# edp1096/toy-spice

Measured on NVIDIA B200. Metric: circuit-timesteps/sec (batched FP64 transient), higher is better.
Workload: dtype f64

## Files before the change

### toy-spice_b200/csrc/device/skeleton.cuh

```cuda
#ifndef TSB_SKELETON_CUH
#define TSB_SKELETON_CUH

#define TSB_MAX_VARYING 128
#define TSB_UC_MAX 32

struct TsbArgs {
    long long n_inst;
    const double* pv[TSB_MAX_VARYING];
    const double* U;
    int analysis;
    int uic;
    double tstart, tstop, tstep, maxstep, minstep;
    int max_iter;
    double abstol, reltol, trtol;
    int out_flags;
    long long cap_rows;
    double* wave;
    double* stats;
    long long* rows;
    int* status;
    long long* counters;
    double* scratch;
    const double* sweep;
    int n_sweep;
// ... 92 lines not shown
    long long inst;
    long long n_rows;
    bool overflow;
    double2* sm;
    int grid_k;
    __device__ __forceinline__ TsbSink(const TsbArgs& a_, long long inst_) : a(a_), inst(inst_), n_rows(0), overflow(false), grid_k(0) {
        sm = reinterpret_cast<double2*>(tsb_smem) + threadIdx.x;
    }
    __device__ __forceinline__ void begin(long long inst_) {
        inst = inst_; n_rows = 0; overflow = false; grid_k = 0;
        if (a.out_flags & TSB_OUT_STATS) {
#pragma unroll
            for (int j = 0; j < NCOL; ++j) {
                sm[(2 * j) * TSB_BLOCK] = make_double2(__longlong_as_double(0x7ff0000000000000LL),
                                                       __longlong_as_double(0xfff0000000000000LL));
                sm[(2 * j + 1) * TSB_BLOCK] = make_double2(0.0, 0.0);
            }
        }
    }
    __device__ __forceinline__ double grid_time(int k) const {
        const double t = __dadd_rn(a.tstart, __dmul_rn((double)(k + 1), a.grid_dt));
        return t < a.tstop ? t : a.tstop;
    }
    __device__ __forceinline__ void emit_grid(const double* row) {
        const double t1 = row[0];
        while (grid_k < a.n_grid) {
            const double tg = grid_time(grid_k);
            if (tg > t1) break;
            double w = 1.0;
            if (n_rows > 0) { const double t0 = sm[1 * TSB_BLOCK].y; w = (tg - t0) / (t1 - t0); }
            double* o = a.wave + ((long long)grid_k * NCOL) * a.n_inst + inst;
            __stcs(o, tg);
#pragma unroll
            for (int j = 1; j < NCOL; ++j) {
                const double v0 = n_rows > 0 ? sm[(2 * j + 1) * TSB_BLOCK].y : row[j];
                __stcs(o + j * a.n_inst, v0 + (row[j] - v0) * w);
            }
            ++grid_k;
        }
    }
    __device__ __forceinline__ void push(const double* row) {
        if (TSB_GRID && (a.out_flags & TSB_OUT_GRID)) emit_grid(row);
        if (a.out_flags & TSB_OUT_WAVE) {
            if (n_rows < a.cap_rows) {
                double* w = a.wave + (n_rows * NCOL) * a.n_inst + inst;
#pragma unroll
                for (int j = 0; j < NCOL; ++j) __stcs(w + j * a.n_inst, row[j]);
            } else overflow = true;
        }
        if (a.out_flags & TSB_OUT_STATS) {
            if (n_rows == 0) sm[0] = make_double2(row[0], row[0]);
            bool grow = !TSB_X_GROW;
#pragma unroll
            for (int j = 1; TSB_X_GROW && j < NCOL; ++j) {
                const double2 mm = sm[(2 * j) * TSB_BLOCK];
                grow |= (row[j] < mm.x) | (row[j] > mm.y);
            }
            if (grow) {
#pragma unroll
                for (int j = 1; j < NCOL; ++j) {
                    const double v = row[j];
                    double2 mm = sm[(2 * j) * TSB_BLOCK];
                    if (TSB_X_STATS_PRED) {
                        double* slot = reinterpret_cast<double*>(&sm[(2 * j) * TSB_BLOCK]);
                        if (v < mm.x) slot[0] = v;
                        if (v > mm.y) slot[1] = v;
                    } else {
                        mm.x = v < mm.x ? v : mm.x;
                        mm.y = v > mm.y ? v : mm.y;
                        sm[(2 * j) * TSB_BLOCK] = mm;
                    }
                }
            }
#pragma unroll
            for (int j = 0; j < NCOL; ++j) {
                double2 sl = sm[(2 * j + 1) * TSB_BLOCK];
                sl.x += row[j];
                sl.y = row[j];
                sm[(2 * j + 1) * TSB_BLOCK] = sl;
            }
        }
        ++n_rows;
    }
    __device__ __forceinline__ void finish(bool ok = true) {
        if (TSB_GRID && (a.out_flags & TSB_OUT_GRID) && ok && n_rows > 0) {
            while (grid_k < a.n_grid) {
                double* o = a.wave + ((long long)grid_k * NCOL) * a.n_inst + inst;
                __stcs(o, grid_time(grid_k));
#pragma unroll
                for (int j = 1; j < NCOL; ++j) __stcs(o + j * a.n_inst, sm[(2 * j + 1) * TSB_BLOCK].y);
                ++grid_k;
            }
        }
        if (a.out_flags & TSB_OUT_STATS) {
#pragma unroll
            for (int j = 0; j < NCOL; ++j) {
                double2 mm = sm[(2 * j) * TSB_BLOCK];
                const double2 sl = sm[(2 * j + 1) * TSB_BLOCK];
                if (j == 0 && n_rows > 0) {
                    const double f = mm.x, l = sl.y;
                    mm.x = f < l ? f : l; mm.y = f < l ? l : f;
                }
                a.stats[(long long)(0 * NCOL + j) * a.n_inst + inst] = mm.x;
                a.stats[(long long)(1 * NCOL + j) * a.n_inst + inst] = mm.y;
                a.stats[(long long)(2 * NCOL + j) * a.n_inst + inst] = sl.x;
                a.stats[(long long)(3 * NCOL + j) * a.n_inst + inst] = sl.y;
            }
        }
        a.rows[inst] = (TSB_GRID && (a.out_flags & TSB_OUT_GRID)) ? (long long)grid_k : n_rows;
    }
};

#ifndef TSB_TGRID
#define TSB_TGRID 0
#endif
#ifndef TSB_X_TG_EARLY
#define TSB_X_TG_EARLY 1
#endif
#define TSB_TG_HDR 3
#define TSB_TG_NO_KEY (-3.0)
template <int NSRC> struct TsbTgLayout { static constexpr int ND = ((TSB_TG_HDR + NSRC + 1) / 2) * 2; };
__device__ __forceinline__ unsigned long long tsb_ld_acquire(const unsigned long long* p) {
    unsigned long long v;
    asm volatile("ld.acquire.gpu.global.u64 %0, [%1];" : "=l"(v) : "l"(p) : "memory");
    return v;
}
__device__ __forceinline__ void tsb_st_release(unsigned long long* p, unsigned long long v) {
    asm volatile("st.release.gpu.global.u64 [%0], %1;" ::"l"(p), "l"(v) : "memory");
}
__device__ __forceinline__ unsigned long long tsb_ld_relaxed(const unsigned long long* p) {
    unsigned long long v;
    asm volatile("ld.relaxed.gpu.global.u64 %0, [%1];" : "=l"(v) : "l"(p) : "memory");
    return v;
}
__device__ __forceinline__ void tsb_fence_acquire() { asm volatile("fence.acq_rel.gpu;" ::: "memory"); }
__device__ __forceinline__ void tsb_prefetch_l1(const void* p) { asm volatile("prefetch.global.L1 [%0];" ::"l"(p)); }
#ifndef TSB_TG_PUBLISH_EVERY
#define TSB_TG_PUBLISH_EVERY 8
#endif
#ifndef TSB_TG_LOOK_EVERY
#define TSB_TG_LOOK_EVERY 16
#endif
#ifndef TSB_TG_CACHED
#define TSB_TG_CACHED 0
#endif
#ifndef TSB_TG_PREFETCH
#define TSB_TG_PREFETCH 0
#endif
#if TSB_TG_CACHED
#define TSB_TG_LD(p) __ldca(p)
#else
#define TSB_TG_LD(p) __ldcg(p)
#endif

template <bool HAVE_KEY = false, bool HAVE_SMALL = false, class Ckt, class Sink>
__device__ __forceinline__ void tsb_accept_step(const TsbArgs& a, Ckt& c, Sink& sink, double& time, double& dt,
                                                double next_time, double lte, TsbTimeKeyer& keyer, double& last_key, double key_in = 0.0,
                                                bool lte_small = false) {
    c.load_state(dt);
    c.update_state();
    time = next_time;
    if (time >= a.tstart) {
        double key = HAVE_KEY ? key_in : keyer.key(time);
        if (key != last_key) {
            double row[Ckt::NCOL_MAX];
            row[0] = time;
            c.signals(row + 1);
            sink.push(row);
            last_key = key;
        }
    }
    if (time < a.tstop && dt < a.maxstep) {
        const double grown = (HAVE_SMALL ? lte_small : lte < a.trtol / 100) ? dt * 2 : dt * 1.1;
        dt = grown < a.maxstep ? grown : a.maxstep;
    }
}

template <class Ckt, class Sink>
__device__ __forceinline__ void tsb_tran_linear(const TsbArgs& a, Ckt& c, Sink& sink, long long& n_acc_out, long long& n_rej_out,
                                                long long& n_sol_tran_out, long long& n_exec_out, int& status, double& fail_at) {
    double time = 0.0, dt = a.minstep;
    double last_key = -1.0;
    TsbTimeKeyer keyer; keyer.reset();
    int n_acc = 0, n_rej = 0, n_bad = 0;
    constexpr int ND = TsbTgLayout<Ckt::NSRC>::ND;
    const bool tg_pub = TSB_TGRID && a.tgrid != nullptr && a.tgrid_role == 1;
    const bool tg_reader = TSB_TGRID && a.tgrid != nullptr && a.tgrid_role == 0;
    int tg_limit = TSB_X_TGLOOK ? 0 : (tg_reader ? 0 : -1);
    int tg_next = tg_reader ? 0 : 0x7fffffff;
#if TSB_X_UNROLL2
#pragma unroll 2
#endif
    while (time < a.tstop) {
        const int k = n_acc + n_rej;
        const double t_tag = time, dt_tag = dt;
        bool look = false;
        if (TSB_TGRID && TSB_X_TGLOOK) {
            if (k == tg_next) {
                const unsigned long long pub = tsb_ld_relaxed(a.tgrid_pub);
                const int lim = pub < (unsigned long long)a.tgrid_cap ? (int)pub : a.tgrid_cap;
                if (lim > k) { tsb_fence_acquire(); tg_limit = lim; tg_next = (lim + TSB_TG_LOOK_EVERY - 1) & ~(TSB_TG_LOOK_EVERY - 1); }
                else tg_next = k + TSB_TG_LOOK_EVERY;
                if (k >= a.tgrid_cap) { tg_limit = 0; tg_next = 0x7fffffff; }
            }
            look = k < tg_limit;
        } else if (TSB_TGRID && tg_limit >= 0) {
            if (k >= tg_limit && (k & (TSB_TG_LOOK_EVERY - 1)) == 0) {
                const unsigned long long pub = tsb_ld_relaxed(a.tgrid_pub);
                const int lim = pub < (unsigned long long)a.tgrid_cap ? (int)pub : a.tgrid_cap;
                if (lim > k) { tsb_fence_acquire(); tg_limit = lim; }
                if (k >= a.tgrid_cap) tg_limit = -1;
            }
            look = k < tg_limit;
            if (TSB_TG_PREFETCH && look) tsb_prefetch_l1(a.tgrid + (long long)k * ND);
        }
#if TSB_X_TGLOOK
        double2 e0, e1;
#else
        double2 e0 = make_double2(0.0, 0.0), e1 = make_double2(0.0, 0.0);
#endif
        if (TSB_TGRID && TSB_X_TG_EARLY && look) {
            const double2* e = reinterpret_cast<const double2*>(a.tgrid + (long long)k * ND);
            e0 = TSB_TG_LD(e); e1 = TSB_TG_LD(e + 1);
        }
        double next_time = time + dt;
        if (next_time > a.tstop) { next_time = a.tstop; dt = next_time - time; }
        __builtin_assume(dt > 0.0);
        const double rdt = tsb_rcp_dt(dt);
        double lte = 0.0;
        bool lte_gt, lte_small;
        if (TSB_X_LTEFLAGS) c.lte_flags(dt, rdt, a.trtol, a.trtol / 100, lte_gt, lte_small);
        else { lte = c.lte(dt, rdt); lte_gt = lte > a.trtol; lte_small = lte < a.trtol / 100; }
        if (lte_gt && dt > a.minstep) {
            if (tg_pub && k < a.tgrid_cap) {
                double2* e = reinterpret_cast<double2*>(a.tgrid + (long long)k * ND);
                __stcg(e, make_double2(t_tag, dt_tag));
                __stcg(e + 1, make_double2(TSB_TG_NO_KEY, 0.0));
                if ((k & (TSB_TG_PUBLISH_EVERY - 1)) == TSB_TG_PUBLISH_EVERY - 1) tsb_st_release(a.tgrid_pub, (unsigned long long)k + 1);
            }
            dt /= 2; ++n_rej; continue;
        }
        double key = 0.0;
        auto mid = [&]() {
            bool hit = false;
            if (TSB_TGRID && look) {
                const double2* e = reinterpret_cast<const double2*>(a.tgrid + (long long)k * ND);
                if (!TSB_X_TG_EARLY) { e0 = TSB_TG_LD(e); e1 = TSB_TG_LD(e + 1); }
                hit = ((__double_as_longlong(e0.x) ^ __double_as_longlong(t_tag)) | (__double_as_longlong(e0.y) ^ __double_as_longlong(dt_tag))) == 0;
                if (!hit) { tg_limit = TSB_X_TGLOOK ? 0 : -1; tg_next = 0x7fffffff; }
                hit = hit && e1.x != TSB_TG_NO_KEY;
                if (hit) {
                    key = e1.x;
                    if (Ckt::SRC_UNIFORM) {
                        c.SV[0] = e1.y;
#pragma unroll
                        for (int j = 1; j < Ckt::NSRC; j += 2) {
                            const double2 sv = TSB_TG_LD(e + 2 + j / 2);
                            c.SV[j] = sv.x;
                            if (j + 1 < Ckt::NSRC) c.SV[j + 1] = sv.y;
                        }
                    }
                }
            }
            if (!hit || !Ckt::SRC_UNIFORM) { if (!c.eval_sources_nb(time)) c.eval_sources(time, 1.0); }
            if (!hit) key = next_time >= a.tstart ? keyer.key_any(next_time) : -2.0;
            if (tg_pub && k < a.tgrid_cap) {
                double2* e = reinterpret_cast<double2*>(a.tgrid + (long long)k * ND);
                __stcg(e, make_double2(t_tag, dt_tag));
                __stcg(e + 1, make_double2(key, c.SV[0]));
#pragma unroll
                for (int j = 1; j < Ckt::NSRC; j += 2) __stcg(e + 2 + j / 2, make_double2(c.SV[j], j + 1 < Ckt::NSRC ? c.SV[j + 1] : 0.0));
                if ((k & (TSB_TG_PUBLISH_EVERY - 1)) == TSB_TG_PUBLISH_EVERY - 1) tsb_st_release(a.tgrid_pub, (unsigned long long)k + 1);
            }
        };
        bool solved;
        if constexpr (Ckt::HAS_TF) solved = c.template assemble_solve_tf<false>(time, dt, rdt, mid);
        else solved = c.template assemble_solve<TSB_MODE_TRAN, false>(TSB_MODE_TRAN, time, dt, rdt, 0.0, mid);
        if (!solved) {
            ++n_bad;
            if (dt > a.minstep) { dt /= 2; ++n_rej; continue; }
            status = TSB_ST_TRAN_FAILED; fail_at = time;
            break;
        }
        tsb_accept_step<true, true>(a, c, sink, time, dt, next_time, lte, keyer, last_key, key, lte_small);
        ++n_acc;
    }
    if (tg_pub) { const int k = n_acc + n_rej; tsb_st_release(a.tgrid_pub, (unsigned long long)(k < a.tgrid_cap ? k : a.tgrid_cap)); }
    n_acc_out += n_acc; n_rej_out += n_rej;
    const int failed = status == TSB_ST_TRAN_FAILED ? 1 : 0;
    n_exec_out += n_acc + (n_bad - failed) + failed;
    n_sol_tran_out += 2LL * (n_acc + n_rej) - n_bad + 2 * failed;
}

#ifndef TSB_X_NLLOOP
#define TSB_X_NLLOOP 1
#endif
template <class Ckt, class Sink>
__device__ __forceinline__ void tsb_tran_nonlinear(const TsbArgs& a, Ckt& c, Sink& sink, bool active, long long& n_acc_out,
                                                   long long& n_rej_out, long long& n_sol_tran_out, long long& n_exec_out,
                                                   int& status, double& fail_at) {
    constexpr int N = Ckt::N;
    double time = 0.0, dt = a.minstep;
    double last_key = -1.0;
    TsbTimeKeyer keyer; keyer.reset();
    int n_acc = 0, n_rej = 0, n_sol = 0;
    bool live = active && time < a.tstop;
    while (__any_sync(0xffffffffu, live)) {
        double next_time = time + dt;
        if (next_time > a.tstop) { next_time = a.tstop; dt = next_time - time; }
        double rdt = 0.0;
        if (live) {
            if (!c.eval_sources_nb(time)) c.eval_sources(time, 1.0);
            rdt = tsb_rcp_dt(dt);
        }
        int iter = 0;
#if TSB_X_NRSTATE
        int nr = live ? 0 : 2;
        while (__any_sync(0xffffffffu, nr == 0)) {
            if (nr == 0) {
                if (iter > 0) c.update_nl(c.xo);
                bool solved;
                if constexpr (Ckt::HAS_TF) solved = c.template assemble_solve_tf<true>(time, dt, rdt, typename Ckt::TsbNoMid());
                else solved = c.template assemble_solve<TSB_MODE_TRAN>(TSB_MODE_TRAN, time, dt, rdt, 0.0);
                ++n_sol;
                if (!solved) nr = 2;
                else {
                    const bool cv = iter > 0 && tsb_converged<N>(c.x, c.xo, a.reltol, a.abstol);
                    if (cv) nr = 1;
                    else {
#pragma unroll
                        for (int i = 1; i <= N; ++i) c.xo[i] = c.x[i];
                        if (++iter >= a.max_iter) nr = 2;
                    }
                }
            }
        }
        const bool fail = nr == 2;
#else
        bool conv = false, fail = false, iterating = live;
        while (__any_sync(0xffffffffu, iterating)) {
            if (iterating) {
                if (iter > 0) c.update_nl(c.xo);
                bool solved;
                if constexpr (Ckt::HAS_TF) solved = c.template assemble_solve_tf<true>(time, dt, rdt, typename Ckt::TsbNoMid());
                else solved = c.template assemble_solve<TSB_MODE_TRAN>(TSB_MODE_TRAN, time, dt, rdt, 0.0);
                ++n_sol;
                if (!solved) fail = true;
                else {
                    if (iter > 0) conv = tsb_converged<N>(c.x, c.xo, a.reltol, a.abstol);
                    if (!conv) {
#pragma unroll
                        for (int i = 1; i <= N; ++i) c.xo[i] = c.x[i];
                        if (++iter >= a.max_iter) fail = true;
                    }
                }
                iterating = !(conv || fail);
            }
        }
#endif
        if (live) {
            if (fail) {
                if (dt > a.minstep) { dt /= 2; ++n_rej; }
                else { status = TSB_ST_TRAN_FAILED; fail_at = time; live = false; }
            } else {
                const double lte = c.lte(dt, rdt);
                if (lte > a.trtol && dt > a.minstep) { dt /= 2; ++n_rej; }
                else {
                    tsb_accept_step(a, c, sink, time, dt, next_time, lte, keyer, last_key);
                    ++n_acc;
                    live = time < a.tstop;
                }
            }
        }
    }
    n_acc_out += n_acc; n_rej_out += n_rej; n_sol_tran_out += n_sol; n_exec_out += n_sol;
}

#ifndef TSB_X_WSYNC
#define TSB_X_WSYNC 1
#endif
template <class Ckt>
__device__ __forceinline__ void tsb_run_optran_instance(const TsbArgs& a, long long inst, bool valid) {
    constexpr int N = Ckt::N;
    constexpr bool LINEAR_LOOP = !Ckt::HAS_NL && (TSB_SKIP_LINEAR_RESOLVE != 0);
    constexpr bool REFILL = Ckt::HAS_NL && (TSB_LANE_REFILL != 0);
    constexpr bool WSYNC = Ckt::HAS_NL && !REFILL && (TSB_X_WSYNC != 0);
    constexpr bool NL_LOOP = WSYNC && (TSB_X_NLLOOP != 0);
    if (!WSYNC && !valid) return;
    Ckt c;
    TsbSink<Ckt::NCOL_MAX> sink(a, inst);

    long long n_acc, n_rej, n_sol_tran, n_sol_op;
    long long n_exec;
    int op_path, status;
    double fail_at;

    enum { PH_OP_START, PH_TRAN_BEGIN, PH_NR, PH_DONE };
    enum { C_MAIN, C_GMIN, C_GFINAL, C_SRC, C_SFINAL, C_TRAN };
    int phase, op_pass, cont, iter, mode, gstep;
    double gmin, sfac, status_dt;
    double time, dt, next_time, rdt;
    double last_key;
    TsbTimeKeyer keyer;
    bool linear_tran;

    auto begin_instance = [&]() {
        c.load(a, inst);
        c.init();
        if constexpr (Ckt::HAS_TF) c.prefactor();
        sink.begin(inst);
        n_acc = n_rej = n_sol_tran = n_sol_op = n_exec = 0;
        op_path = 0; status = TSB_ST_OK; fail_at = 0.0;
        phase = (a.analysis == TSB_AN_TRAN && a.uic) ? PH_TRAN_BEGIN : PH_OP_START;
        op_pass = 0; cont = C_MAIN; iter = 0; mode = TSB_MODE_OP; gstep = 0;
        gmin = 0.0; sfac = 0.0; status_dt = 0.0;
        time = 0.0; dt = a.minstep; next_time = 0.0; rdt = 0.0;
        last_key = -1.0; keyer.reset();
        linear_tran = false;
        if (phase == PH_TRAN_BEGIN && !(time < a.tstop)) phase = PH_DONE;
        if ((LINEAR_LOOP || NL_LOOP) && phase == PH_TRAN_BEGIN) { linear_tran = true; phase = PH_DONE; }
    };
    auto finish_instance = [&]() {
        if (sink.overflow && status == TSB_ST_OK) status = TSB_ST_OVERFLOW;
        if (a.analysis == TSB_AN_OP) a.rows[inst] = sink.n_rows; else sink.finish(status == TSB_ST_OK);
        a.status[inst] = status;
        a.counters[0 * a.n_inst + inst] = n_acc;
        a.counters[1 * a.n_inst + inst] = n_rej;
        a.counters[2 * a.n_inst + inst] = n_sol_tran;
        a.counters[3 * a.n_inst + inst] = n_sol_op;
        a.counters[4 * a.n_inst + inst] = op_path;
        a.counters[5 * a.n_inst + inst] = __double_as_longlong(fail_at);
        a.counters[6 * a.n_inst + inst] = n_exec;
        a.counters[7 * a.n_inst + inst] = sink.n_rows;
    };
    bool done = !valid;
    bool pend = false;
    bool conv = false, fail = false;
    phase = PH_DONE;
    if (valid) begin_instance();
// ... 270 lines not shown
```

### toy-spice_b200/csrc/runtime.cpp

```cpp
#include <cuda_runtime.h>
#include <dlfcn.h>
#include <sys/stat.h>
#include <unistd.h>
#include <atomic>
#include <cmath>
#include <cstdio>
#include <cstdlib>
#include <cstring>
#include <fstream>
#include <memory>
#include <mutex>
#include <sstream>
#include "tsb_internal.hpp"
#include "hostlu.hpp"

namespace tsb {
cudaError_t launch_fp64_peak(double* scratch, int blocks, int iters, cudaStream_t s);
cudaError_t launch_totals(const long long* counters, long long n_inst, unsigned long long* totals, int sms, cudaStream_t s);
cudaError_t launch_fill_i64(long long* p, long long n, long long v, int sms, cudaStream_t s);
cudaError_t launch_summary(const double* stats, long long n_inst, int ncol, double* partial, int blocks_x, cudaStream_t s);
cudaError_t launch_lu_warp(const double* A, const double* b, double* x, int* status, long long n_inst, int n, const int* prow,
                           const int* pcol, int strict, int sms, cudaStream_t s);
cudaError_t launch_clu_warp(const double* A, const double* b, double* x, int* status, long long n_inst, int n, const int* prow,
                            const int* pcol, int strict, int sms, cudaStream_t s);
// ... 919 lines not shown
    if ((d.kind == TSB_V || d.kind == TSB_I) && d.src_type() == TSB_SRC_PWL)
        return fail(b->ctx, TSB_E_UNSUPPORTED, "PWL tables are not sweepable");
    *flat = d.p_off + param;
    return TSB_OK;
}
static int claim_slot(tsb_batch* b, int flat) {
    if (b->var_slot[flat] >= 0) return b->var_slot[flat];
    b->varying[flat] = 1;
    b->var_slot[flat] = (int)b->slot_ptr.size();
    b->slot_ptr.push_back(nullptr);
    b->slot_owned.push_back(0);
    b->slot_stage.push_back(nullptr);
    b->slot_staged.push_back(nullptr);
    return b->var_slot[flat];
}
static int set_param_host(tsb_batch* b, int dev, int param, const double* values, bool staged) {
    int flat = 0, rc = param_index(b, dev, param, &flat);
    if (rc != TSB_OK) return rc;
    if (!values) return TSB_E_INVALID;
    int slot = claim_slot(b, flat);
    if (!b->ctx) return TSB_OK;
    tsb_ctx* ctx = b->ctx;
    CU(ctx, cudaSetDevice(ctx->device));
    const size_t bytes = (size_t)b->n_inst * sizeof(double);
    if (!b->slot_owned[slot]) {
        double* p = nullptr;
        CU(ctx, cudaMalloc(&p, bytes));
        b->slot_ptr[slot] = p; b->slot_owned[slot] = 1;
    }
    const double* src = values;
    if (staged) {
        if (!b->slot_stage[slot]) {
            CU(ctx, cudaMallocHost((void**)&b->slot_stage[slot], bytes));
            CU(ctx, cudaEventCreateWithFlags(&b->slot_staged[slot], cudaEventDisableTiming));
        } else CU(ctx, cudaEventSynchronize(b->slot_staged[slot]));
        memcpy(b->slot_stage[slot], values, bytes);
        src = b->slot_stage[slot];
    }
    cudaStream_t up = ctx->stream;
    cudaStreamCaptureStatus cap = cudaStreamCaptureStatusNone;
    if (cudaStreamIsCapturing(ctx->stream, &cap) != cudaSuccess) { cudaGetLastError(); cap = cudaStreamCaptureStatusNone; }
    const bool beside = cap == cudaStreamCaptureStatusNone;
    if (beside) {
        if (!ctx->upload_stream) CU(ctx, cudaStreamCreateWithFlags(&ctx->upload_stream, cudaStreamNonBlocking));
        up = ctx->upload_stream;
        if (b->ev_launched) CU(ctx, cudaStreamWaitEvent(up, b->ev_launched, 0));
    }
    CU(ctx, cudaMemcpyAsync(b->slot_ptr[slot], src, bytes, cudaMemcpyHostToDevice, up));
    if (staged) CU(ctx, cudaEventRecord(b->slot_staged[slot], up));
    if (beside) {
        if (!b->ev_params) CU(ctx, cudaEventCreateWithFlags(&b->ev_params, cudaEventDisableTiming));
        CU(ctx, cudaEventRecord(b->ev_params, up));
        b->params_pending = true;
    }
    return TSB_OK;
}
int tsb_batch_set_param(tsb_batch* b, int dev, int param, const double* values) { return set_param_host(b, dev, param, values, true); }
int tsb_batch_set_param_async(tsb_batch* b, int dev, int param, const double* values) { return set_param_host(b, dev, param, values, false); }
int tsb_batch_set_param_dev(tsb_batch* b, int dev, int param, uint64_t dev_ptr) {
    int flat = 0, rc = param_index(b, dev, param, &flat);
    if (rc != TSB_OK) return rc;
    if (!dev_ptr) return TSB_E_INVALID;
    int slot = claim_slot(b, flat);
    if (b->slot_owned[slot]) { cudaFree(b->slot_ptr[slot]); b->slot_owned[slot] = 0; }
    b->slot_ptr[slot] = (double*)(uintptr_t)dev_ptr;
    return TSB_OK;
}
int tsb_batch_set_param_uniform(tsb_batch* b, int dev, int param, double value) {
    int flat = 0, rc = param_index(b, dev, param, &flat);
    if (rc != TSB_OK) return rc;
    if (b->varying[flat]) return fail(b->ctx, TSB_E_INVALID, "parameter already set per instance");
    b->uniform[flat] = value;
    return TSB_OK;
}

int tsb_run_op(tsb_batch* b, const tsb_opts* opts) {
    int rc = check_batch(b); if (rc != TSB_OK) return rc;
    tsb_ctx* ctx = b->ctx;
    tsb_opts o = resolve(opts, b->plan->p);
    o.coop_parts = 0;
    CU(ctx, cudaSetDevice(ctx->device));
    KernelModule* m = nullptr;
    if ((rc = get_module(b, o, -1, &m)) != TSB_OK) return rc;
    if ((rc = alloc_results(b, TSB_AN_OP, TSB_OUT_WAVE, 1, 0)) != TSB_OK) return rc;
    TsbArgsHost a;
    if ((rc = fill_common(b, o, a)) != TSB_OK) return rc;
    a.analysis = TSB_AN_OP;
    return launch(b, o, m->optran, a, b->plan->p.has_nonlinear && o.lane_refill != 0, m->min_blocks);
}

int tsb_run_tran(tsb_batch* b, double tstart, double tstop, double tstep, double tmax, int uic, int out_flags,
                 int64_t wave_cap_rows, const tsb_opts* opts) {
    int rc = check_batch(b); if (rc != TSB_OK) return rc;
    tsb_ctx* ctx = b->ctx;
    if (!(tstop > 0) || !(tstep > 0)) return fail(ctx, TSB_E_INVALID, "tstop and tstep must be positive");
    if (!(out_flags & (TSB_OUT_WAVE | TSB_OUT_STATS | TSB_OUT_GRID))) return fail(ctx, TSB_E_INVALID, "no output selected");
    if ((out_flags & TSB_OUT_WAVE) && (out_flags & TSB_OUT_GRID)) return fail(ctx, TSB_E_INVALID, "TSB_OUT_WAVE and TSB_OUT_GRID share the waveform buffer: select one");
    if ((out_flags & TSB_OUT_WAVE) && wave_cap_rows <= 0) return fail(ctx, TSB_E_INVALID, "wave_cap_rows must be positive");
    tsb_opts o = resolve(opts, b->plan->p);
    if (tstep > tstop / 300) tstep = tstop / 300;
    double minstep = tstep / 50.0;
    if (tmax == 0) tmax = tstep;
    double grid_dt = 0.0; int64_t n_grid = 0;
    if (out_flags & TSB_OUT_GRID) {
        out_flags |= TSB_OUT_STATS;
        grid_dt = o.grid_dt > 0 ? o.grid_dt : tstep;
        double span = tstop - tstart;
        if (!(span > 0) || !(grid_dt > 0)) return fail(ctx, TSB_E_INVALID, "TSB_OUT_GRID needs tstart < tstop and a positive grid spacing");
        double q = span / grid_dt;
        if (q > 1e7) return fail(ctx, TSB_E_INVALID, "TSB_OUT_GRID: more than 1e7 grid points");
        n_grid = (int64_t)floor(q * (1.0 + 1e-12) + 1e-9);
        if (n_grid < 1) n_grid = 1;
        wave_cap_rows = n_grid;
    }
    CU(ctx, cudaSetDevice(ctx->device));
    if (const char* ce = getenv("TSB_COOP")) { if (*ce) o.coop_parts = atoi(ce); }
    if (o.coop_parts < 0) {
        const Plan& cpl = b->plan->p;
        o.coop_parts = 0;
        if (!cpl.has_bjt && !cpl.has_mutual && !o.strict_fp && !(out_flags & TSB_OUT_GRID) && o.skip_linear_resolve && !o.lane_refill) {
            if (cpl.n() >= TSB_COOP_AUTO_MIN_N)
                for (int pick : {2, 4, 8}) {
                    if (!cpl.coop.count(pick)) continue;
                    const int nx = cpl.coop.at(pick).nx, nown = cpl.coop.at(pick).nown_max;
                    if (((size_t)4 * nown * 32 * pick + (size_t)2 * pick * nx * 32) * sizeof(double) <= 110 * 1024) { o.coop_parts = pick; break; }
                }
        }
    }
    if (o.coop_parts != 0) {
        const Plan& cpl = b->plan->p;
        if (o.coop_parts != 2 && o.coop_parts != 4 && o.coop_parts != 8) return fail(ctx, TSB_E_INVALID, "coop_parts must be -1, 0, 2, 4 or 8");
        if (cpl.has_bjt || cpl.has_mutual) return fail(ctx, TSB_E_UNSUPPORTED, "coop_parts: circuits with BJTs or mutual couplings run thread-per-circuit");
        if (!cpl.coop.count(o.coop_parts)) return fail(ctx, TSB_E_UNSUPPORTED, "coop_parts: the netlist has no partition into that many sub-circuits (tsb_plan_coop_info)");
        if (o.strict_fp) return fail(ctx, TSB_E_UNSUPPORTED, "coop_parts: the nested-dissection order is a re-association, not available in the strict build");
        if (out_flags & TSB_OUT_GRID) return fail(ctx, TSB_E_UNSUPPORTED, "coop_parts: TSB_OUT_GRID is not available on the cooperative mapping");
        if (!o.skip_linear_resolve || o.lane_refill) return fail(ctx, TSB_E_UNSUPPORTED, "coop_parts needs skip_linear_resolve = 1 and lane_refill = 0");
        if (o.min_blocks <= 0) o.min_blocks = 2;
    } else fit_block_to_shared_memory(o, b->plan->p.num_columns(TSB_AN_TRAN), out_flags);
    KernelModule* m = nullptr;
    b->grid_kernel = (out_flags & TSB_OUT_GRID) != 0;
    std::string autokey;
    rc = get_module(b, o, -1, &m, &autokey);
    if (rc != TSB_OK) { b->grid_kernel = false; return rc; }
    if ((rc = alloc_results(b, TSB_AN_TRAN, out_flags, (out_flags & (TSB_OUT_WAVE | TSB_OUT_GRID)) ? wave_cap_rows : 0, 0)) != TSB_OK) return rc;
    TsbArgsHost a;
    if ((rc = fill_common(b, o, a)) != TSB_OK) return rc;
    a.analysis = TSB_AN_TRAN; a.uic = uic;
    a.tstart = tstart; a.tstop = tstop; a.tstep = tstep; a.maxstep = tmax; a.minstep = minstep;
    a.grid_dt = grid_dt; a.n_grid = (int)n_grid;
    const bool persistent = b->plan->p.has_nonlinear && o.lane_refill != 0;
    const char* tune_env = getenv("TSB_AUTOTUNE");
    cudaStreamCaptureStatus cap = cudaStreamCaptureStatusNone;
    if (cudaStreamIsCapturing(ctx->stream, &cap) != cudaSuccess) { cudaGetLastError(); cap = cudaStreamCaptureStatusNone; }
    if (o.coop_parts == 0 && o.min_blocks <= 0 && !autokey.empty() && b->n_inst >= TSB_TUNE_MIN_INSTANCES && !ctx->tuned.count(autokey) &&
        !(tune_env && *tune_env == '0') && cap == cudaStreamCaptureStatusNone) {
        rc = autotune_min_blocks(b, o, autokey, m->min_blocks, a, persistent);
        if (rc == TSB_OK) rc = get_module(b, o, -1, &m);
        if (rc != TSB_OK) { b->grid_kernel = false; return rc; }
    }
    b->grid_kernel = false;
    b->tgrid_used = 0;
    const Plan& pl = b->plan->p;
    if (o.coop_parts > 0) {
        if (!m->coop) return fail(ctx, TSB_E_COMPILE, "cooperative kernel missing from the module");
        const CoopPlan& cp = pl.coop.at(o.coop_parts);
        if (!b->d_coop_state) CU(ctx, cudaMalloc(&b->d_coop_state, (size_t)(pl.n_state + pl.n() + 1) * b->n_inst * sizeof(double)));
        a.coop_state = b->d_coop_state;
        TsbArgsHost a1 = a;
        a1.out_flags = 0;
        if ((rc = launch(b, o, m->optran, a1, false, m->min_blocks)) != TSB_OK) return rc;
        const int nx = cp.nx, nown = cp.nown_max;
        const int groups = 1, block = 32 * cp.parts * groups;
        const size_t smem = ((size_t)4 * nown * block + (size_t)groups * 2 * cp.parts * nx * 32) * sizeof(double);
        if (smem > 227 * 1024) return fail(ctx, TSB_E_UNSUPPORTED, "coop_parts: the statistics of one block do not fit in shared memory");
        if (smem > 48 * 1024) CU(ctx, cudaFuncSetAttribute((const void*)m->coop, cudaFuncAttributeMaxDynamicSharedMemorySize, (int)smem));
        long long blocks = (a.n_run + 32 * groups - 1) / (32 * groups);
        if (blocks > 0x7fffffffLL) blocks = 0x7fffffffLL;
        if (blocks < 1) blocks = 1;
        void* kargs[] = {&a};
        CU(ctx, cudaLaunchKernel((const void*)m->coop, dim3((unsigned)blocks), dim3((unsigned)block), kargs, smem, ctx->stream));
        ++ctx->launches;
        return note_launched(b);
    }
    const bool tg_possible = !pl.has_nonlinear && o.skip_linear_resolve != 0 && o.share_time_grid != 0 && !persistent;
    if (tg_possible && (o.share_time_grid > 0 || b->n_inst >= TSB_TGRID_MIN_INSTANCES)) {
        if ((rc = launch_pilot(b, o, m->optran, a)) != TSB_OK) return rc;
    }
    rc = launch(b, o, m->optran, a, persistent, m->min_blocks);
    if (rc == TSB_OK && b->tgrid_used) {
        CU(ctx, cudaEventRecord(ctx->ev_join, ctx->pilot_stream));
        CU(ctx, cudaStreamWaitEvent(ctx->stream, ctx->ev_join, 0));
        if ((rc = note_launched(b)) != TSB_OK) return rc;
    }
    return rc;
}

static int run_dc_impl(tsb_batch* b, int src_dev, double start, double stop, double inc, int src2_dev, double start2, double stop2,
                       double inc2, int out_flags, const tsb_opts* opts) {
    int rc = check_batch(b); if (rc != TSB_OK) return rc;
    tsb_ctx* ctx = b->ctx;
    const Plan& p = b->plan->p;
    const bool nested = src2_dev != -1;
    auto is_vsrc = [&](int d) { return d >= 0 && d < (int)p.devs.size() && p.devs[d].kind == TSB_V; };
    if (!is_vsrc(src_dev) || (nested && !is_vsrc(src2_dev)))
        return fail(ctx, TSB_E_INVALID, nested ? "source not found" : "source not found");
    if (!(inc > 0) || (nested && !(inc2 > 0))) return fail(ctx, TSB_E_INVALID, "sweep increment must be positive");
    if (out_flags & TSB_OUT_GRID) return fail(ctx, TSB_E_INVALID, "TSB_OUT_GRID applies to transient analysis only");
    if (!(out_flags & (TSB_OUT_WAVE | TSB_OUT_STATS))) return fail(ctx, TSB_E_INVALID, "no output selected");
    std::vector<double> s1, s2;
    for (double v = start; v <= stop; v += inc) { s1.push_back(v); if (s1.size() > (1u << 24)) break; }
    if (nested) for (double v = start2; v <= stop2; v += inc2) { s2.push_back(v); if (s2.size() > (1u << 24)) break; }
    std::vector<double> sweep, sweep2;
    if (!nested) sweep = s1;
    else {
        if ((double)s1.size() * (double)s2.size() > (double)(1u << 24)) return fail(ctx, TSB_E_INVALID, "nested sweep: more than 2^24 points");
        for (double v1 : s1) for (double v2 : s2) { sweep.push_back(v1); sweep2.push_back(v2); }
    }
    tsb_opts o = resolve(opts, b->plan->p);
    o.coop_parts = 0;
    fit_block_to_shared_memory(o, p.num_columns(nested ? (int)TSB_AN_DC2 : (int)TSB_AN_DC), out_flags);
    CU(ctx, cudaSetDevice(ctx->device));
    auto dc_param_of = [&](int d) {
        const Dev& sd = p.devs[d];
        const int st = sd.src_type();
        return (st == TSB_SRC_DC || st == TSB_SRC_SIN) ? sd.p_off : -1;
    };
    const int dc_param = dc_param_of(src_dev), dc_param2 = nested ? dc_param_of(src2_dev) : -1;
    if ((dc_param >= 0 && b->varying[dc_param]) || (dc_param2 >= 0 && b->varying[dc_param2]))
        return fail(ctx, TSB_E_INVALID, "the swept source value is set per instance");
    const int an = nested ? (int)TSB_AN_DC2 : (int)TSB_AN_DC;
    KernelModule* m = nullptr;
    b->dc_nested = nested; b->dc_param2 = dc_param2;
    rc = get_module(b, o, dc_param, &m);
    b->dc_nested = false; b->dc_param2 = -1;
    if (rc != TSB_OK) return rc;
    if ((rc = alloc_results(b, an, out_flags, (out_flags & TSB_OUT_WAVE) ? (int64_t)sweep.size() : 0, (int)sweep.size())) != TSB_OK) return rc;
    TsbArgsHost a;
    if ((rc = fill_common(b, o, a)) != TSB_OK) return rc;
    if (!sweep.empty()) {
        CU(ctx, cudaMemcpyAsync(b->d_sweep, sweep.data(), sweep.size() * sizeof(double), cudaMemcpyHostToDevice, ctx->stream));
        if (nested) CU(ctx, cudaMemcpyAsync(b->d_sweep2, sweep2.data(), sweep2.size() * sizeof(double), cudaMemcpyHostToDevice, ctx->stream));
    }
    CU(ctx, cudaStreamSynchronize(ctx->stream));
    a.analysis = TSB_AN_DC; a.sweep = b->d_sweep; a.sweep2 = b->d_sweep2; a.n_sweep = (int)sweep.size();
    return launch(b, o, m->dc, a);
}
int tsb_run_dc(tsb_batch* b, int src_dev, double start, double stop, double inc, int out_flags, const tsb_opts* opts) {
    return run_dc_impl(b, src_dev, start, stop, inc, -1, 0, 0, 0, out_flags, opts);
}
int tsb_run_dc2(tsb_batch* b, int src1_dev, double start1, double stop1, double inc1, int src2_dev, double start2, double stop2,
                double inc2, int out_flags, const tsb_opts* opts) {
    if (src2_dev < 0) return fail(b ? b->ctx : nullptr, TSB_E_INVALID, "source not found");
    return run_dc_impl(b, src1_dev, start1, stop1, inc1, src2_dev, start2, stop2, inc2, out_flags, opts);
}

int tsb_run_ac(tsb_batch* b, int sweep_type, int n_points, double fstart, double fstop, int out_flags, const tsb_opts* opts) {
    int rc = check_batch(b); if (rc != TSB_OK) return rc;
    tsb_ctx* ctx = b->ctx;
    const Plan& p = b->plan->p;
    if (p.has_nonlinear)
        return fail(ctx, TSB_E_UNSUPPORTED, "AC analysis of a circuit with nonlinear devices: the reference takes their small-signal values from an "
                                             "operating point it solves on a complex matrix with a real-indexed right-hand side (matrix/circuit.go:99-105, "
                                             ":126-150); that state is an artefact of the un-vendored sparse module and is not reproduced");
    if (sweep_type < 0 || sweep_type > 2 || n_points < 1 || n_points > (1 << 20)) return fail(ctx, TSB_E_INVALID, "invalid sweep type or number of points");
    if (out_flags & TSB_OUT_GRID) return fail(ctx, TSB_E_INVALID, "TSB_OUT_GRID applies to transient analysis only");
    if (!(out_flags & (TSB_OUT_WAVE | TSB_OUT_STATS))) return fail(ctx, TSB_E_INVALID, "no output selected");
    std::vector<double> f;
    ac_frequency_points(sweep_type, n_points, fstart, fstop, f);
    tsb_opts o = resolve(opts, p);
    o.coop_parts = 0;
    fit_block_to_shared_memory(o, b->plan->p.num_columns(TSB_AN_AC), out_flags);
    CU(ctx, cudaSetDevice(ctx->device));
    KernelModule* m = nullptr;
    if ((rc = get_module(b, o, -1, &m)) != TSB_OK) return rc;
    if ((rc = alloc_results(b, TSB_AN_AC, out_flags, (out_flags & TSB_OUT_WAVE) ? (int64_t)n_points : 0, n_points)) != TSB_OK) return rc;
    TsbArgsHost a;
    if ((rc = fill_common(b, o, a)) != TSB_OK) return rc;
    CU(ctx, cudaMemcpyAsync(b->d_sweep, f.data(), f.size() * sizeof(double), cudaMemcpyHostToDevice, ctx->stream));
    CU(ctx, cudaStreamSynchronize(ctx->stream));
    a.analysis = TSB_AN_AC; a.sweep = b->d_sweep; a.n_sweep = n_points;
    return launch(b, o, m->ac, a);
}

int tsb_batch_stamp_dev(tsb_batch* b, int mode, double time, double dt, double gmin, uint64_t A_dev, uint64_t b_dev, const tsb_opts* opts) {
    int rc = check_batch(b); if (rc != TSB_OK) return rc;
    tsb_ctx* ctx = b->ctx;
    if (!A_dev || !b_dev || (mode != 0 && mode != 1)) return fail(ctx, TSB_E_INVALID, "tsb_batch_stamp_dev: mode must be 0 (OP) or 1 (transient), outputs non-null");
    tsb_opts o = resolve(opts, b->plan->p);
    o.coop_parts = 0;
    CU(ctx, cudaSetDevice(ctx->device));
    KernelModule* m = nullptr;
    if ((rc = get_module(b, o, -1, &m)) != TSB_OK) return rc;
    TsbArgsHost a;
    if ((rc = fill_common(b, o, a)) != TSB_OK) return rc;
    a.analysis = mode; a.tstart = time; a.tstep = dt; a.minstep = gmin;
    a.wave = (double*)(uintptr_t)A_dev; a.stats = (double*)(uintptr_t)b_dev;
    a.out_flags = 0;
    const int n = b->plan->p.n();
    const size_t per_thread = (size_t)(((n * n + n) | 1)) * sizeof(double);
    int block = o.block_size > 0 ? o.block_size : 128;
    int staged_threads = (int)(200 * 1024 / per_thread) / 32 * 32;
    if (staged_threads > block) staged_threads = block;
    const char* env = getenv("TSB_STAMP_DIRECT");
    const bool staged = staged_threads >= 32 && !(env && *env == '1');
    cudaKernel_t kern = staged ? m->stamp_staged : m->stamp;
    size_t smem = 0;
    if (staged) {
        block = staged_threads;
        smem = (size_t)block * per_thread;
        if (smem > 48 * 1024) CU(ctx, cudaFuncSetAttribute((const void*)kern, cudaFuncAttributeMaxDynamicSharedMemorySize, (int)smem));
    }
    long long blocks = (b->n_inst + block - 1) / block;
    long long resident = (long long)ctx->sms * 32;
    if (blocks > resident) blocks = resident;
    void* kargs[] = {&a};
    CU(ctx, cudaLaunchKernel((const void*)kern, dim3((unsigned)blocks), dim3((unsigned)block), kargs, smem, ctx->stream));
    ++ctx->launches;
    return note_launched(b);
}

int tsb_batch_set_order(tsb_batch* b, const int64_t* perm) {
    int rc = check_batch(b); if (rc != TSB_OK) return rc;
    tsb_ctx* ctx = b->ctx;
    CU(ctx, cudaSetDevice(ctx->device));
    if (!perm) { CU(ctx, cudaStreamSynchronize(ctx->stream)); cudaFree(b->d_order); b->d_order = nullptr; return TSB_OK; }
    std::vector<char> seen((size_t)b->n_inst, 0);
    for (int64_t i = 0; i < b->n_inst; ++i) {
        if (perm[i] < 0 || perm[i] >= b->n_inst || seen[(size_t)perm[i]]) return fail(ctx, TSB_E_INVALID, "tsb_batch_set_order: not a permutation of 0..n_inst-1");
        seen[(size_t)perm[i]] = 1;
    }
    if (!b->d_order) CU(ctx, cudaMalloc(&b->d_order, (size_t)b->n_inst * sizeof(long long)));
    static_assert(sizeof(long long) == sizeof(int64_t), "order entries are 64-bit");
    CU(ctx, cudaMemcpyAsync(b->d_order, perm, (size_t)b->n_inst * sizeof(long long), cudaMemcpyHostToDevice, ctx->stream));
    CU(ctx, cudaStreamSynchronize(ctx->stream));
    return TSB_OK;
}

int tsb_batch_sync(tsb_batch* b) {
    int rc = check_batch(b); if (rc != TSB_OK) return rc;
    CU(b->ctx, cudaSetDevice(b->ctx->device));
// ... 255 lines not shown
```

Before: 122.3 billion.

## Add hit-only fast loop for time-grid readers and pilot before autotune

Splits the linear transient step into an attempt function and adds a specialised HIT_ONLY path for reader lanes. While the pilot's shared time grid matches, this path skips source evaluation, key computation and publish logic, and it falls back to the general path on the first miss. The host now also runs the pilot before autotuning, so the tuning runs see the shared-grid behaviour. It adds test-only macros for fault injection, more code size and some register pressure, and an extra pilot launch during autotune.

```diff
diff --git a/toy-spice_b200/csrc/device/skeleton.cuh b/toy-spice_b200/csrc/device/skeleton.cuh
--- a/toy-spice_b200/csrc/device/skeleton.cuh
+++ b/toy-spice_b200/csrc/device/skeleton.cuh
@@ -268,6 +268,16 @@
 #else
 #define TSB_TG_LD(p) __ldcg(p)
 #endif
+#ifdef TSB_TG_TEST_DT_AT
+#define TSB_TG_DT_TAG(k, d) ((k) == TSB_TG_TEST_DT_AT ? __longlong_as_double(__double_as_longlong(d) ^ 1) : (d))
+#define TSB_TG_VAL_TAG(k, v) ((k) == TSB_TG_TEST_DT_AT ? (v) + 1.0 : (v))
+#else
+#define TSB_TG_DT_TAG(k, d) (d)
+#define TSB_TG_VAL_TAG(k, v) (v)
+#endif
+#ifndef TSB_TG_TEST_ALL_PILOT
+#define TSB_TG_TEST_ALL_PILOT 0
+#endif
 
 template <bool HAVE_KEY = false, bool HAVE_SMALL = false, class Ckt, class Sink>
 __device__ __forceinline__ void tsb_accept_step(const TsbArgs& a, Ckt& c, Sink& sink, double& time, double& dt,
@@ -292,115 +302,160 @@
     }
 }
 
+#ifndef TSB_X_HITLOOP
+#ifdef TSB_FAST_DIV
+#define TSB_X_HITLOOP 0
+#else
+#define TSB_X_HITLOOP 1
+#endif
+#endif
+
+struct TsbLinState {
+    double time, dt, last_key;
+    TsbTimeKeyer keyer;
+    int n_acc, n_rej, n_bad;
+    int tg_limit, tg_next;
+};
+#define TSB_ATT_NEXT 0
+#define TSB_ATT_FAIL 1
+#define TSB_ATT_GENERAL 2
+
+template <bool HIT_ONLY, class Ckt, class Sink>
+__device__ __forceinline__ int tsb_tran_linear_attempt(const TsbArgs& a, Ckt& c, Sink& sink, TsbLinState& s, bool tg_pub,
+                                                       int& status, double& fail_at) {
+    constexpr int ND = TsbTgLayout<Ckt::NSRC>::ND;
+    tg_pub = !HIT_ONLY && tg_pub;
+    double& time = s.time;
+    double& dt = s.dt;
+    const int k = s.n_acc + s.n_rej;
+    const double t_tag = time, dt_tag = dt;
+    bool look = false;
+    if (TSB_TGRID && TSB_X_TGLOOK) {
+        if (k == s.tg_next) {
+            const unsigned long long pub = tsb_ld_relaxed(a.tgrid_pub);
+            const int lim = pub < (unsigned long long)a.tgrid_cap ? (int)pub : a.tgrid_cap;
+            if (lim > k) { tsb_fence_acquire(); s.tg_limit = lim; s.tg_next = (lim + TSB_TG_LOOK_EVERY - 1) & ~(TSB_TG_LOOK_EVERY - 1); }
+            else s.tg_next = k + TSB_TG_LOOK_EVERY;
+            if (k >= a.tgrid_cap) { s.tg_limit = 0; s.tg_next = 0x7fffffff; }
+        }
+        look = k < s.tg_limit;
+    } else if (TSB_TGRID && s.tg_limit >= 0) {
+        if (k >= s.tg_limit && (k & (TSB_TG_LOOK_EVERY - 1)) == 0) {
+            const unsigned long long pub = tsb_ld_relaxed(a.tgrid_pub);
+            const int lim = pub < (unsigned long long)a.tgrid_cap ? (int)pub : a.tgrid_cap;
+            if (lim > k) { tsb_fence_acquire(); s.tg_limit = lim; }
+            if (k >= a.tgrid_cap) s.tg_limit = -1;
+        }
+        look = k < s.tg_limit;
+        if (TSB_TG_PREFETCH && look) tsb_prefetch_l1(a.tgrid + (long long)k * ND);
+    }
+    if (HIT_ONLY && !look) return TSB_ATT_GENERAL;
+#ifdef TSB_TG_TEST_HOLD_AT
+    if (tg_pub && k == TSB_TG_TEST_HOLD_AT) for (int i = 0; i < 1000; ++i) __nanosleep(1000);
+#endif
+#if TSB_X_TGLOOK
+    double2 e0, e1;
+#else
+    double2 e0 = make_double2(0.0, 0.0), e1 = make_double2(0.0, 0.0);
+#endif
+    if (TSB_TGRID && TSB_X_TG_EARLY && look) {
+        const double2* e = reinterpret_cast<const double2*>(a.tgrid + (long long)k * ND);
+        e0 = TSB_TG_LD(e); e1 = TSB_TG_LD(e + 1);
+    }
+    double next_time = time + dt;
+    if (next_time > a.tstop) { next_time = a.tstop; dt = next_time - time; }
+    __builtin_assume(dt > 0.0);
+    const double rdt = tsb_rcp_dt(dt);
+    double lte = 0.0;
+    bool lte_gt, lte_small;
+    if (TSB_X_LTEFLAGS) c.lte_flags(dt, rdt, a.trtol, a.trtol / 100, lte_gt, lte_small);
+    else { lte = c.lte(dt, rdt); lte_gt = lte > a.trtol; lte_small = lte < a.trtol / 100; }
+    if (lte_gt && dt > a.minstep) {
+        if (tg_pub && k < a.tgrid_cap) {
+            double2* e = reinterpret_cast<double2*>(a.tgrid + (long long)k * ND);
+            __stcg(e, make_double2(t_tag, TSB_TG_DT_TAG(k, dt_tag)));
+            __stcg(e + 1, make_double2(TSB_TG_NO_KEY, 0.0));
+            if ((k & (TSB_TG_PUBLISH_EVERY - 1)) == TSB_TG_PUBLISH_EVERY - 1) tsb_st_release(a.tgrid_pub, (unsigned long long)k + 1);
+        }
+        dt /= 2; ++s.n_rej; return TSB_ATT_NEXT;
+    }
+    double key = 0.0;
+    bool hit = false;
+    auto mid = [&]() {
+        if (TSB_TGRID && look) {
+            const double2* e = reinterpret_cast<const double2*>(a.tgrid + (long long)k * ND);
+            if (!TSB_X_TG_EARLY) { e0 = TSB_TG_LD(e); e1 = TSB_TG_LD(e + 1); }
+            hit = ((__double_as_longlong(e0.x) ^ __double_as_longlong(t_tag)) | (__double_as_longlong(e0.y) ^ __double_as_longlong(dt_tag))) == 0;
+            if (!hit) { s.tg_limit = TSB_X_TGLOOK ? 0 : -1; s.tg_next = 0x7fffffff; }
+            hit = hit && e1.x != TSB_TG_NO_KEY;
+            if (hit || HIT_ONLY) {
+                key = e1.x;
+                if (Ckt::SRC_UNIFORM) {
+                    c.SV[0] = e1.y;
+#pragma unroll
+                    for (int j = 1; j < Ckt::NSRC; j += 2) {
+                        const double2 sv = TSB_TG_LD(e + 2 + j / 2);
+                        c.SV[j] = sv.x;
+                        if (j + 1 < Ckt::NSRC) c.SV[j + 1] = sv.y;
+                    }
+                }
+            }
+        }
+        if (HIT_ONLY) {
+            if (!Ckt::SRC_UNIFORM) { if (!c.eval_sources_nb(time)) c.eval_sources(time, 1.0); }
+            return;
+        }
+        if (!hit || !Ckt::SRC_UNIFORM) { if (!c.eval_sources_nb(time)) c.eval_sources(time, 1.0); }
+        if (!hit) key = next_time >= a.tstart ? s.keyer.key_any(next_time) : -2.0;
+        if (tg_pub && k < a.tgrid_cap) {
+            double2* e = reinterpret_cast<double2*>(a.tgrid + (long long)k * ND);
+            __stcg(e, make_double2(t_tag, TSB_TG_DT_TAG(k, dt_tag)));
+            __stcg(e + 1, make_double2(TSB_TG_VAL_TAG(k, key), TSB_TG_VAL_TAG(k, c.SV[0])));
+#pragma unroll
+            for (int j = 1; j < Ckt::NSRC; j += 2) __stcg(e + 2 + j / 2, make_double2(c.SV[j], j + 1 < Ckt::NSRC ? c.SV[j + 1] : 0.0));
+            if ((k & (TSB_TG_PUBLISH_EVERY - 1)) == TSB_TG_PUBLISH_EVERY - 1) tsb_st_release(a.tgrid_pub, (unsigned long long)k + 1);
+        }
+    };
+    bool solved;
+    if constexpr (Ckt::HAS_TF) solved = c.template assemble_solve_tf<false>(time, dt, rdt, mid);
+    else solved = c.template assemble_solve<TSB_MODE_TRAN, false>(TSB_MODE_TRAN, time, dt, rdt, 0.0, mid);
+    if (HIT_ONLY && !hit) { dt = dt_tag; return TSB_ATT_GENERAL; }
+    if (!solved) {
+        ++s.n_bad;
+        if (dt > a.minstep) { dt /= 2; ++s.n_rej; return TSB_ATT_NEXT; }
+        status = TSB_ST_TRAN_FAILED; fail_at = time;
+        return TSB_ATT_FAIL;
+    }
+    tsb_accept_step<true, true>(a, c, sink, time, dt, next_time, lte, s.keyer, s.last_key, key, lte_small);
+    ++s.n_acc;
+    return TSB_ATT_NEXT;
+}
+
 template <class Ckt, class Sink>
 __device__ __forceinline__ void tsb_tran_linear(const TsbArgs& a, Ckt& c, Sink& sink, long long& n_acc_out, long long& n_rej_out,
                                                 long long& n_sol_tran_out, long long& n_exec_out, int& status, double& fail_at) {
-    double time = 0.0, dt = a.minstep;
-    double last_key = -1.0;
-    TsbTimeKeyer keyer; keyer.reset();
-    int n_acc = 0, n_rej = 0, n_bad = 0;
-    constexpr int ND = TsbTgLayout<Ckt::NSRC>::ND;
-    const bool tg_pub = TSB_TGRID && a.tgrid != nullptr && a.tgrid_role == 1;
-    const bool tg_reader = TSB_TGRID && a.tgrid != nullptr && a.tgrid_role == 0;
-    int tg_limit = TSB_X_TGLOOK ? 0 : (tg_reader ? 0 : -1);
-    int tg_next = tg_reader ? 0 : 0x7fffffff;
+    TsbLinState s;
+    s.time = 0.0; s.dt = a.minstep;
+    s.last_key = -1.0;
+    s.keyer.reset();
+    s.n_acc = s.n_rej = s.n_bad = 0;
+    const bool tg_pub = TSB_TGRID && a.tgrid != nullptr && (a.tgrid_role == 1 || TSB_TG_TEST_ALL_PILOT);
+    const bool tg_reader = TSB_TGRID && a.tgrid != nullptr && a.tgrid_role == 0 && !TSB_TG_TEST_ALL_PILOT;
+    s.tg_limit = TSB_X_TGLOOK ? 0 : (tg_reader ? 0 : -1);
+    s.tg_next = tg_reader ? 0 : 0x7fffffff;
+    const bool hit_loop = TSB_TGRID && TSB_X_HITLOOP && tg_reader;
 #if TSB_X_UNROLL2
 #pragma unroll 2
 #endif
-    while (time < a.tstop) {
-        const int k = n_acc + n_rej;
-        const double t_tag = time, dt_tag = dt;
-        bool look = false;
-        if (TSB_TGRID && TSB_X_TGLOOK) {
-            if (k == tg_next) {
-                const unsigned long long pub = tsb_ld_relaxed(a.tgrid_pub);
-                const int lim = pub < (unsigned long long)a.tgrid_cap ? (int)pub : a.tgrid_cap;
-                if (lim > k) { tsb_fence_acquire(); tg_limit = lim; tg_next = (lim + TSB_TG_LOOK_EVERY - 1) & ~(TSB_TG_LOOK_EVERY - 1); }
-                else tg_next = k + TSB_TG_LOOK_EVERY;
-                if (k >= a.tgrid_cap) { tg_limit = 0; tg_next = 0x7fffffff; }
-            }
-            look = k < tg_limit;
-        } else if (TSB_TGRID && tg_limit >= 0) {
-            if (k >= tg_limit && (k & (TSB_TG_LOOK_EVERY - 1)) == 0) {
-                const unsigned long long pub = tsb_ld_relaxed(a.tgrid_pub);
-                const int lim = pub < (unsigned long long)a.tgrid_cap ? (int)pub : a.tgrid_cap;
-                if (lim > k) { tsb_fence_acquire(); tg_limit = lim; }
-                if (k >= a.tgrid_cap) tg_limit = -1;
-            }
-            look = k < tg_limit;
-            if (TSB_TG_PREFETCH && look) tsb_prefetch_l1(a.tgrid + (long long)k * ND);
-        }
-#if TSB_X_TGLOOK
-        double2 e0, e1;
-#else
-        double2 e0 = make_double2(0.0, 0.0), e1 = make_double2(0.0, 0.0);
-#endif
-        if (TSB_TGRID && TSB_X_TG_EARLY && look) {
-            const double2* e = reinterpret_cast<const double2*>(a.tgrid + (long long)k * ND);
-            e0 = TSB_TG_LD(e); e1 = TSB_TG_LD(e + 1);
-        }
-        double next_time = time + dt;
-        if (next_time > a.tstop) { next_time = a.tstop; dt = next_time - time; }
-        __builtin_assume(dt > 0.0);
-        const double rdt = tsb_rcp_dt(dt);
-        double lte = 0.0;
-        bool lte_gt, lte_small;
-        if (TSB_X_LTEFLAGS) c.lte_flags(dt, rdt, a.trtol, a.trtol / 100, lte_gt, lte_small);
-        else { lte = c.lte(dt, rdt); lte_gt = lte > a.trtol; lte_small = lte < a.trtol / 100; }
-        if (lte_gt && dt > a.minstep) {
-            if (tg_pub && k < a.tgrid_cap) {
-                double2* e = reinterpret_cast<double2*>(a.tgrid + (long long)k * ND);
-                __stcg(e, make_double2(t_tag, dt_tag));
-                __stcg(e + 1, make_double2(TSB_TG_NO_KEY, 0.0));
-                if ((k & (TSB_TG_PUBLISH_EVERY - 1)) == TSB_TG_PUBLISH_EVERY - 1) tsb_st_release(a.tgrid_pub, (unsigned long long)k + 1);
-            }
-            dt /= 2; ++n_rej; continue;
-        }
-        double key = 0.0;
-        auto mid = [&]() {
-            bool hit = false;
-            if (TSB_TGRID && look) {
-                const double2* e = reinterpret_cast<const double2*>(a.tgrid + (long long)k * ND);
-                if (!TSB_X_TG_EARLY) { e0 = TSB_TG_LD(e); e1 = TSB_TG_LD(e + 1); }
-                hit = ((__double_as_longlong(e0.x) ^ __double_as_longlong(t_tag)) | (__double_as_longlong(e0.y) ^ __double_as_longlong(dt_tag))) == 0;
-                if (!hit) { tg_limit = TSB_X_TGLOOK ? 0 : -1; tg_next = 0x7fffffff; }
-                hit = hit && e1.x != TSB_TG_NO_KEY;
-                if (hit) {
-                    key = e1.x;
-                    if (Ckt::SRC_UNIFORM) {
-                        c.SV[0] = e1.y;
-#pragma unroll
-                        for (int j = 1; j < Ckt::NSRC; j += 2) {
-                            const double2 sv = TSB_TG_LD(e + 2 + j / 2);
-                            c.SV[j] = sv.x;
-                            if (j + 1 < Ckt::NSRC) c.SV[j + 1] = sv.y;
-                        }
-                    }
-                }
-            }
-            if (!hit || !Ckt::SRC_UNIFORM) { if (!c.eval_sources_nb(time)) c.eval_sources(time, 1.0); }
-            if (!hit) key = next_time >= a.tstart ? keyer.key_any(next_time) : -2.0;
-            if (tg_pub && k < a.tgrid_cap) {
-                double2* e = reinterpret_cast<double2*>(a.tgrid + (long long)k * ND);
-                __stcg(e, make_double2(t_tag, dt_tag));
-                __stcg(e + 1, make_double2(key, c.SV[0]));
-#pragma unroll
-                for (int j = 1; j < Ckt::NSRC; j += 2) __stcg(e + 2 + j / 2, make_double2(c.SV[j], j + 1 < Ckt::NSRC ? c.SV[j + 1] : 0.0));
-                if ((k & (TSB_TG_PUBLISH_EVERY - 1)) == TSB_TG_PUBLISH_EVERY - 1) tsb_st_release(a.tgrid_pub, (unsigned long long)k + 1);
-            }
-        };
-        bool solved;
-        if constexpr (Ckt::HAS_TF) solved = c.template assemble_solve_tf<false>(time, dt, rdt, mid);
-        else solved = c.template assemble_solve<TSB_MODE_TRAN, false>(TSB_MODE_TRAN, time, dt, rdt, 0.0, mid);
-        if (!solved) {
-            ++n_bad;
-            if (dt > a.minstep) { dt /= 2; ++n_rej; continue; }
-            status = TSB_ST_TRAN_FAILED; fail_at = time;
-            break;
-        }
-        tsb_accept_step<true, true>(a, c, sink, time, dt, next_time, lte, keyer, last_key, key, lte_small);
-        ++n_acc;
-    }
+    while (s.time < a.tstop) {
+        if (hit_loop && (TSB_X_TGLOOK ? s.tg_next != 0x7fffffff : s.tg_limit >= 0)) {
+            int r = TSB_ATT_NEXT;
+            while (r == TSB_ATT_NEXT && s.time < a.tstop) r = tsb_tran_linear_attempt<true>(a, c, sink, s, false, status, fail_at);
+            if (r != TSB_ATT_GENERAL) break;
+        }
+        if (tsb_tran_linear_attempt<false>(a, c, sink, s, tg_pub, status, fail_at) == TSB_ATT_FAIL) break;
+    }
+    const int n_acc = s.n_acc, n_rej = s.n_rej, n_bad = s.n_bad;
     if (tg_pub) { const int k = n_acc + n_rej; tsb_st_release(a.tgrid_pub, (unsigned long long)(k < a.tgrid_cap ? k : a.tgrid_cap)); }
     n_acc_out += n_acc; n_rej_out += n_rej;
     const int failed = status == TSB_ST_TRAN_FAILED ? 1 : 0;
diff --git a/toy-spice_b200/csrc/runtime.cpp b/toy-spice_b200/csrc/runtime.cpp
--- a/toy-spice_b200/csrc/runtime.cpp
+++ b/toy-spice_b200/csrc/runtime.cpp
@@ -1095,15 +1095,24 @@
     const char* tune_env = getenv("TSB_AUTOTUNE");
     cudaStreamCaptureStatus cap = cudaStreamCaptureStatusNone;
     if (cudaStreamIsCapturing(ctx->stream, &cap) != cudaSuccess) { cudaGetLastError(); cap = cudaStreamCaptureStatusNone; }
+    const Plan& pl = b->plan->p;
+    const bool tg_possible = !pl.has_nonlinear && o.skip_linear_resolve != 0 && o.share_time_grid != 0 && !persistent;
+    const bool tg_run = tg_possible && (o.share_time_grid > 0 || b->n_inst >= TSB_TGRID_MIN_INSTANCES);
+    b->tgrid_used = 0;
     if (o.coop_parts == 0 && o.min_blocks <= 0 && !autokey.empty() && b->n_inst >= TSB_TUNE_MIN_INSTANCES && !ctx->tuned.count(autokey) &&
         !(tune_env && *tune_env == '0') && cap == cudaStreamCaptureStatusNone) {
+        if (tg_run) {
+            if ((rc = launch_pilot(b, o, m->optran, a)) != TSB_OK) { b->grid_kernel = false; return rc; }
+            if (b->tgrid_used) {
+                CU(ctx, cudaEventRecord(ctx->ev_join, ctx->pilot_stream));
+                CU(ctx, cudaStreamWaitEvent(ctx->stream, ctx->ev_join, 0));
+            }
+        }
         rc = autotune_min_blocks(b, o, autokey, m->min_blocks, a, persistent);
         if (rc == TSB_OK) rc = get_module(b, o, -1, &m);
         if (rc != TSB_OK) { b->grid_kernel = false; return rc; }
     }
     b->grid_kernel = false;
-    b->tgrid_used = 0;
-    const Plan& pl = b->plan->p;
     if (o.coop_parts > 0) {
         if (!m->coop) return fail(ctx, TSB_E_COMPILE, "cooperative kernel missing from the module");
         const CoopPlan& cp = pl.coop.at(o.coop_parts);
@@ -1125,10 +1134,7 @@
         ++ctx->launches;
         return note_launched(b);
     }
-    const bool tg_possible = !pl.has_nonlinear && o.skip_linear_resolve != 0 && o.share_time_grid != 0 && !persistent;
-    if (tg_possible && (o.share_time_grid > 0 || b->n_inst >= TSB_TGRID_MIN_INSTANCES)) {
-        if ((rc = launch_pilot(b, o, m->optran, a)) != TSB_OK) return rc;
-    }
+    if (tg_run && (rc = launch_pilot(b, o, m->optran, a)) != TSB_OK) return rc;
     rc = launch(b, o, m->optran, a, persistent, m->min_blocks);
     if (rc == TSB_OK && b->tgrid_used) {
         CU(ctx, cudaEventRecord(ctx->ev_join, ctx->pilot_stream));
```

Result: no change. 123.1 billion (median of 6 runs) (+0.7%).
